# bioinformatics-centre/kaiju

Hardware: AMD Instinct MI355X
Metric: classified reads/sec (150 bp) (higher is better)
Workload: dtype u64

## Files before the change

### kaiju_amd/csrc/capi.hip

```cpp
#include <algorithm>
#include <chrono>
#include <cstdio>
#include <cstring>
#include <memory>
#include <thread>

#include "capi_internal.h"
#include "host_tables.h"
#include "kj_flow.h"
#include "taxonomy.h"
#include "exact_pass.h"
#include "kj_format.h"
#ifdef KJ_GREEDY3
#include "kj_greedy3.h"
#endif

using namespace kj;

constexpr uint32_t kLocDeferRows = 8;

__device__ __forceinline__ void load_tables(ConstTables &s_ct, const ConstTables *g_ct) {
  const uint32_t *src = reinterpret_cast<const uint32_t *>(g_ct);
  uint32_t *dst = reinterpret_cast<uint32_t *>(&s_ct);
  for (uint32_t i = threadIdx.x; i < sizeof(ConstTables) / 4; i += kBlock) dst[i] = src[i];
// ... 113 lines not shown
      }
      F[k].flags = fl;
    }
    b.meta[r].nfrag = nf | pending;
    uint64_t *h8 = reinterpret_cast<uint64_t *>(b.hits + r);
    for (int x = 0; x < (int)(sizeof(Hit) / 8); x++) h8[x] = 0;
  }
}
__global__ void __launch_bounds__(kBlock)
k_seg_apply_list(const ConstTables *__restrict__ g_ct, Params p, Batch b, SegQueue sq, const uint32_t *seglist,
                 const uint32_t *segcount, uint32_t *err) {
  __shared__ ConstTables s_ct;
  load_tables(s_ct, g_ct);
  const uint32_t n = *segcount;
  uint32_t e = 0;
  for (uint32_t i = blockIdx.x * kBlock + threadIdx.x; i < n; i += gridDim.x * kBlock) seg_apply_mem(s_ct, p, b, sq, seglist[i], &e);
  if (e) atomicOr(err, e);
}

#ifdef KJ_POST_WAVES
#define KJ_POST_BOUNDS __launch_bounds__(256, KJ_POST_WAVES)
#else
#define KJ_POST_BOUNDS __launch_bounds__(256)
#endif
template <bool LCA>
__global__ void KJ_POST_BOUNDS
k_mem_post1(const Stage1Tables *__restrict__ g_t, DevIndex ix, Params p, Batch b, DevTaxonomy t, CompactHit *__restrict__ compact, int lazy,
            uint32_t *seglist, uint32_t *segcount, uint32_t *todo, uint32_t *todocount) {
  __shared__ __attribute__((aligned(16))) Stage1Tables s_t;
  __shared__ __attribute__((aligned(4))) uint8_t s_cnt[256 * kS1CntStride];
  if (lazy) {
    const uint4 *src = reinterpret_cast<const uint4 *>(g_t);
    uint4 *dst = reinterpret_cast<uint4 *>(&s_t);
    for (uint32_t i = threadIdx.x; i < sizeof(Stage1Tables) / 16; i += 256) dst[i] = src[i];
    __syncthreads();
  }
  const uint32_t r = blockIdx.x * 256 + threadIdx.x;
  bool need = false, later = false;
  if (r < b.n_reads) {
    Hit *h = b.hits + r;
    const uint32_t v = lazy ? h->reserved : 0u;
    if (v != 0) {
      h->reserved = 0;
#ifndef KJ_POST_NOTRIG
      need = lazy_seg_needed(s_t, p, b, r, h, v, nullptr, s_cnt + threadIdx.x * kS1CntStride);
#endif
    }
    if (!need) {
      if (h->flags & kHitRetry) later = true;
#ifdef KJ_POST_NOLOCATE
      else if (LCA) { CompactHit ch; ch.lca = 0; ch.best = h->best; ch.info = 0; compact[r] = ch; }
#else
      else if (!mem_locate_read<false>(ix, p, h, kLocDeferRows)) later = true;
      else if (LCA) compact[r] = compact_hit(t, *h);
#endif
    }
  }
  const uint32_t lane = threadIdx.x & 63u;
  {
    const uint64_t m = __ballot(need);
    if (m) {
      const uint32_t leader = (uint32_t)__builtin_ctzll(m);
      uint32_t base = 0;
      if (lane == leader) base = atomicAdd(segcount, (uint32_t)__popcll(m));
      base = (uint32_t)__shfl((int)base, (int)leader, 64);
      if (need) seglist[base + (uint32_t)__popcll(m & ((1ull << lane) - 1ull))] = r;
    }
  }
  {
    const bool td = need || later;
    const uint64_t m = __ballot(td);
    if (m) {
      const uint32_t leader = (uint32_t)__builtin_ctzll(m);
      uint32_t base = 0;
      if (lane == leader) base = atomicAdd(todocount, (uint32_t)__popcll(m));
      base = (uint32_t)__shfl((int)base, (int)leader, 64);
      if (td) todo[base + (uint32_t)__popcll(m & ((1ull << lane) - 1ull))] = r;
    }
  }
}
template <bool LCA>
__global__ void __launch_bounds__(256)
k_mem_post2(DevIndex ix, Params p, Batch b, DevTaxonomy t, CompactHit *__restrict__ compact, const uint32_t *__restrict__ todo,
            const uint32_t *__restrict__ todocount) {
  const uint32_t n = *todocount;
  for (uint32_t i = blockIdx.x * 256 + threadIdx.x; i < n; i += gridDim.x * 256) {
    const uint32_t r = todo[i];
    Hit *h = b.hits + r;
    if (!mem_locate_read<false>(ix, p, h, kLocDeferRows)) mem_locate_read<false, true>(ix, p, h);
    if (LCA) compact[r] = compact_hit(t, *h);
  }
}

__global__ void __launch_bounds__(kFragBlock)
k_fragments_protein(const ConstTables *__restrict__ g_ct, Params p, SegTables st, Batch b, SegQueue sq, uint32_t *err) {
  __shared__ ConstTables s_ct;
  __shared__ int32_t s_entg[17];
  __shared__ uint8_t s_code[256];
  if (threadIdx.x < 17) s_entg[threadIdx.x] = st.ent_g32[threadIdx.x];
  {
    const uint32_t *src = reinterpret_cast<const uint32_t *>(g_ct);
    uint32_t *dst = reinterpret_cast<uint32_t *>(&s_ct);
    for (uint32_t i = threadIdx.x; i < sizeof(ConstTables) / 4; i += kFragBlock) dst[i] = src[i];
    for (uint32_t i = threadIdx.x; i < 256; i += kFragBlock) s_code[i] = 0;
    __syncthreads();
    if (threadIdx.x < 20) protein_code_entry(s_ct, threadIdx.x, s_code);
    __syncthreads();
// ... 418 lines not shown
    for (int x = threadIdx.x & 63; x < 2 + 3 * PS_N; x += 64) s_prof[threadIdx.x >> 6][x] = 0;
    gx.prof = s_prof[threadIdx.x >> 6];
    if ((threadIdx.x & 63) == 0) { gx.prof[0] = __builtin_readcyclecounter(); gx.prof[1] = PS_HEAD; }
  }
#endif
  greedy_lane3<COUNT>(ix, s_ct, p, sq, b, wl, gx);
}
__global__ void __launch_bounds__(kG3Threads, 2)
k_greedy3(DevIndex ix, const ConstTables *__restrict__ g_ct, Params p, SegQueue sq, Batch b, WorkList wl, GreedyArrays2 ga, uint32_t split) {
  greedy3_body<false>(ix, g_ct, p, sq, b, wl, ga, split);
}
__global__ void __launch_bounds__(kG3Threads, 2)
k_greedy3_count(DevIndex ix, const ConstTables *__restrict__ g_ct, Params p, SegQueue sq, Batch b, WorkList wl, GreedyArrays2 ga, uint32_t split) {
  greedy3_body<true>(ix, g_ct, p, sq, b, wl, ga, split);
}

#endif

static_assert(sizeof(ConstTables) % 4 == 0, "ConstTables is copied as dwords");
static_assert(sizeof(Hit) == sizeof(kaiju_gpu_hit), "hit layout");

static thread_local std::string tl_error;
int fail(int code, const std::string &msg) { tl_error = msg; return code; }

extern "C" int kaiju_gpu_abi_version(void) { return KAIJU_GPU_ABI_VERSION; }
extern "C" const char *kaiju_gpu_last_error(void) { return tl_error.c_str(); }
extern "C" void kj_set_last_error(const char *msg) { tl_error = msg ? msg : ""; }
extern "C" const char *kaiju_gpu_strerror(int status) {
  switch (status) {
    case KAIJU_GPU_OK: return "ok";
    case KAIJU_GPU_ERR_ARG: return "bad argument";
    case KAIJU_GPU_ERR_IO: return "I/O error";
    case KAIJU_GPU_ERR_FORMAT: return "unrecognised file content";
    case KAIJU_GPU_ERR_NO_DEVICE: return "no usable HIP device (this library has no CPU path)";
    case KAIJU_GPU_ERR_HIP: return "HIP runtime error";
    case KAIJU_GPU_ERR_NOMEM: return "out of memory";
    case KAIJU_GPU_ERR_UNSUPPORTED: return "parameter not supported by the kernels";
    case KAIJU_GPU_ERR_INDEX_BUG: return "index triggers a latent bug of the reference";
    default: return "unknown status";
  }
}
extern "C" int kaiju_gpu_device_count(void) {
  int n = 0;
  if (hipGetDeviceCount(&n) != hipSuccess) return 0;
  return n;
}
int no_device() {
  int ndev = 0;
  if (hipGetDeviceCount(&ndev) != hipSuccess || ndev <= 0) return fail(KAIJU_GPU_ERR_NO_DEVICE, "hipGetDeviceCount found no device");
  return KAIJU_GPU_OK;
}

__global__ void __launch_bounds__(256)
k_lca(DevTaxonomy t, const Hit *__restrict__ hits, uint32_t n, CompactHit *__restrict__ out) {
  const uint32_t r = blockIdx.x * 256 + threadIdx.x;
  if (r >= n) return;
  out[r] = compact_hit(t, hits[r]);
}
int launch_lca(hipStream_t s, const kaiju_gpu_taxonomy *t, const kaiju_gpu_hit *d_hits, uint32_t n, kaiju_gpu_compact *d_out) {
  hipLaunchKernelGGL(k_lca, dim3((n + 255) / 256), dim3(256), 0, s, t->dev, reinterpret_cast<const Hit *>(d_hits), n,
                     reinterpret_cast<CompactHit *>(d_out));
  KJ_HIP(hipGetLastError());
  return KAIJU_GPU_OK;
}

int ensure(DevBuf &b, size_t bytes) {
  if (bytes <= b.cap) return 0;
  if (b.p) { KJ_HIP(hipFree(b.p)); b.p = nullptr; b.cap = 0; }
  const size_t want = bytes + bytes / 8 + 256;
  KJ_HIP(hipMalloc(&b.p, want));
  b.cap = want;
  return 0;
}

extern "C" void kaiju_gpu_default_params(kaiju_gpu_params *p, int mode) {
  if (!p) return;
  p->mode = mode ? 1 : 0;
  p->min_fragment_length = 11;
  p->mismatches = 3;
  p->min_score = 65;
  p->seed_length = 7;
  p->seg = 1;
  p->use_evalue = mode ? 1 : 0;
  p->min_evalue = 0.01;
  p->max_matches_SI = 20;
  p->max_match_ids = 20;
  p->input_is_protein = 0;
}

extern "C" int kaiju_gpu_create(kaiju_gpu_ctx **out, const kaiju_gpu_index *ix, const kaiju_gpu_params *p) {
  return guarded([&]() -> int {
  if (!out || !ix || !p) return fail(KAIJU_GPU_ERR_ARG, "NULL argument");
  *out = nullptr;
  if (p->mode != 0 && p->mode != 1) return fail(KAIJU_GPU_ERR_ARG, "mode must be 0 (MEM) or 1 (GREEDY)");
  if (p->min_fragment_length < 1 || p->min_fragment_length > 10000)
    return fail(KAIJU_GPU_ERR_UNSUPPORTED, "min_fragment_length out of range");
  if (p->mode == 1 && p->mismatches > (uint32_t)kMaxMismatch)
    return fail(KAIJU_GPU_ERR_UNSUPPORTED, "more than 8 mismatches are not supported");
  if (p->mode == 1 && p->seed_length < 1) return fail(KAIJU_GPU_ERR_ARG, "seed_length must be >= 1");
  if (p->max_match_ids > 20 || p->max_matches_SI > 64 || p->max_matches_SI < 1)
    return fail(KAIJU_GPU_ERR_UNSUPPORTED, "max_match_ids <= 20 and 1 <= max_matches_SI <= 64 required");
  std::unique_ptr<kaiju_gpu_ctx> c(new kaiju_gpu_ctx());
  c->ix = ix;
  c->params = *p;
  c->kp.mode = p->mode; c->kp.m = p->min_fragment_length; c->kp.mismatches = p->mismatches;
  c->kp.min_score = p->min_score; c->kp.seed_length = p->seed_length; c->kp.seg = p->seg ? 1 : 0;
  c->kp.max_matches_SI = p->max_matches_SI; c->kp.max_match_ids = p->max_match_ids;
  if (const char *e = getenv("KAIJU_GPU_DEBUG")) c->kp.debug = (uint32_t)atoi(e);
  if (const char *e = getenv("KAIJU_GPU_EXACT_PASS")) c->exact_pass = atoi(e) != 0;
  if (const char *e = getenv("KAIJU_GPU_MEM_LANE")) c->mem_v1 = !strcmp(e, "v1");
  if (const char *e = getenv("KAIJU_GPU_VERBOSE_LANE")) c->verbose_v1 = !strcmp(e, "v1");
  c->dump_frags = getenv("KAIJU_GPU_DUMP_FRAGS");
  if (const char *e = getenv("KAIJU_GPU_STAGE1")) { c->stage1_old = !strcmp(e, "old"); c->stage1_lane = !strcmp(e, "lane"); }
  if (const char *e = getenv("KAIJU_GPU_LAZY_SEG")) c->lazy_seg = atoi(e) != 0;
// ... 379 lines not shown
      g2.bestv = nullptr; g2.vb = vb;
      if (c->verbose) {
        if ((rc = ensure(c->vb_bestv, lanes_g2 * 64 * sizeof(GBestV)))) return rc;
        g2.bestv = static_cast<GBestV *>(c->vb_bestv.p);
      }
    }
    call_mark("launch_batch: Greedy scratch in place");
    if (plan.run) {
      const dim3 grid(c->blocks_main);
      const bool counting = plan.inst == FlowInst::Counting;
      switch (plan.lane) {
        case FlowLane::Greedy2Wide:
          if (plan.inst == FlowInst::Verbose) hipLaunchKernelGGL(k_greedy2_wide_vb, grid, blk, kGreedy2Lds, s, ix->dev, ix->d_ct, p_lane, sq, b, wl_main, g2);
          else if (counting) hipLaunchKernelGGL(k_greedy2_wide_count, grid, blk, kGreedy2Lds, s, ix->dev, ix->d_ct, p_lane, sq, b, wl_main, g2);
          else hipLaunchKernelGGL(k_greedy2_wide, grid, blk, kGreedy2Lds, s, ix->dev, ix->d_ct, p_lane, sq, b, wl_main, g2);
          break;
#ifdef KJ_GREEDY3
        case FlowLane::Greedy3:
          if (counting) hipLaunchKernelGGL(k_greedy3_count, dim3(c->n_cu), dim3(c->g3_threads), 0, s, ix->dev, ix->d_ct, p_lane, sq, b, wl_main, g2, c->g3_split);
          else hipLaunchKernelGGL(k_greedy3, dim3(c->n_cu), dim3(c->g3_threads), 0, s, ix->dev, ix->d_ct, p_lane, sq, b, wl_main, g2, c->g3_split);
          break;
#else
        case FlowLane::Greedy3:
#endif
        case FlowLane::Greedy2:
          if (plan.inst == FlowInst::Verbose) hipLaunchKernelGGL(k_greedy2_vb, grid, blk, kGreedy2Lds, s, ix->dev, ix->d_ct, p_lane, sq, b, wl_main, g2);
          else if (counting) hipLaunchKernelGGL(k_greedy2_count, grid, blk, kGreedy2Lds, s, ix->dev, ix->d_ct, p_lane, sq, b, wl_main, g2);
          else hipLaunchKernelGGL(k_greedy2, grid, blk, kGreedy2Lds, s, ix->dev, ix->d_ct, p_lane, sq, b, wl_main, g2);
          break;
        case FlowLane::GreedyV1:
          hipLaunchKernelGGL(k_greedy, grid, blk, 0, s, ix->dev, ix->d_ct, p, sq, b, wl_main, ga, vb);
          break;
        default: break;
      }
      KJ_HIP(hipGetLastError());
      KJ_HIP(hipEventRecord(c->ev[3], s));
      hipLaunchKernelGGL(k_greedy_retry, dim3(c->blocks_retry), blk, 0, s, ix->dev, ix->d_ct, p, sq, b, wl_retry, gr, vb);
      KJ_HIP(hipGetLastError());
      if (plan.mem_verbose) {
        hipLaunchKernelGGL(pick_greedy_verbose(lane_wide), grid_reads, dim3(256), 0, s, ix->dev, p, b, vb);
        KJ_HIP(hipGetLastError());
      }
      launch_locate(c, s, plan.locate, p, b, loc_list, cnt + kCntLocListGreedy);
      KJ_HIP(hipGetLastError());
      if (plan.exact_pass) {
        xp.g_pool = gr.pool; xp.g_ord = gr.ord; xp.g_matches = gr.matches; xp.g_best = gr.best; xp.g_bestv = gr.bestv;
        xp.g_pool_cap = gr.pool_cap; xp.g_match_cap = gr.match_cap; xp.blocks_search = c->blocks_retry;
        xp.vb = vb;
        KJ_HIP(kj_launch_exact_pass(xp));
      }
    } else KJ_HIP(hipEventRecord(c->ev[3], s));
  }
  if (plan.lca) {
    hipLaunchKernelGGL(k_lca, dim3((n + 255) / 256), dim3(256), 0, s, tax->dev, reinterpret_cast<const Hit *>(d_out), n,
                       reinterpret_cast<CompactHit *>(d_compact));
    KJ_HIP(hipGetLastError());
  }
  KJ_HIP(hipEventRecord(c->ev[4], s));
  c->ev_valid = true;
  c->last_n = n;
  if (const char *dump = c->dump_frags) {
    KJ_HIP(hipStreamSynchronize(s));
    std::vector<ReadMeta> hm(n);
    KJ_HIP(hipMemcpy(hm.data(), c->meta.p, (size_t)n * sizeof(ReadMeta), hipMemcpyDeviceToHost));
    std::vector<uint8_t> hp(c->pep.cap);
    KJ_HIP(hipMemcpy(hp.data(), c->pep.p, c->pep.cap, hipMemcpyDeviceToHost));
    std::vector<uint8_t> hf(c->frags.cap);
    KJ_HIP(hipMemcpy(hf.data(), c->frags.p, c->frags.cap, hipMemcpyDeviceToHost));
    const Frag *F = reinterpret_cast<const Frag *>(hf.data());
    if (FILE *fp = fopen(dump, "a")) {
      const char *alpha = ix->info.alphabet;
      for (uint32_t r = 0; r < n; r++) {
        fprintf(fp, "#\n");
        for (uint32_t k = 0; k < (hm[r].nfrag & ~kNfragSegPending); k++) {
          const Frag &f = F[hm[r].frag + k];
          fprintf(fp, "%u:", f.key);
          for (uint32_t x = 0; x < f.len; x++) fputc(alpha[hp[hm[r].pep + f.start + x] % 21], fp);
          fprintf(fp, "\n");
        }
      }
      fclose(fp);
    }
  }
  return KAIJU_GPU_OK;
}

extern "C" int kaiju_gpu_classify_batch_device(kaiju_gpu_ctx *ctx, const void *d_seqs, uint64_t seq_bytes,
                                               const uint64_t *d_off, uint32_t n_reads, int paired,
                                               kaiju_gpu_hit *d_out, void *stream) {
  return guarded([&]() -> int {
  if (!ctx || (!d_seqs && seq_bytes) || !d_off || (!d_out && n_reads)) return fail(KAIJU_GPU_ERR_ARG, "NULL argument");
  KJ_HIP(hipSetDevice(ctx->ix->device));
  hipStream_t s = stream ? static_cast<hipStream_t>(stream) : ctx->stream;
  return launch_batch(ctx, d_seqs, seq_bytes, d_off, n_reads, paired, ctx->max_read_len, d_out, s);
  });
}

int classify_host_buffers(kaiju_gpu_ctx *ctx, const char *seqs, const uint64_t *off, uint32_t n_reads, int paired,
                          const kaiju_gpu_taxonomy *tax) {
  KJ_HIP(hipSetDevice(ctx->ix->device));
  if (off[0] != 0) return fail(KAIJU_GPU_ERR_ARG, "off[0] must be 0");
  const uint64_t seq_bytes = off[2 * (uint64_t)n_reads];
  uint32_t max_len = 0;
  for (uint64_t i = 0; i < 2 * (uint64_t)n_reads; i++) {
    if (off[i + 1] < off[i]) return fail(KAIJU_GPU_ERR_ARG, "offsets must be non-decreasing");
    const uint64_t l = off[i + 1] - off[i];
    if (l > 0x3fffffffull) return fail(KAIJU_GPU_ERR_UNSUPPORTED, "read longer than 2^30");
    if (l > max_len) max_len = (uint32_t)l;
  }
// ... 37 lines not shown
  });
}

extern "C" int kaiju_gpu_set_max_read_length(kaiju_gpu_ctx *ctx, uint32_t max_read_len) {
  if (!ctx || max_read_len == 0 || max_read_len > 0x3fffffffu) return fail(KAIJU_GPU_ERR_ARG, "bad max_read_len");
  ctx->max_read_len = max_read_len;
  return KAIJU_GPU_OK;
}

extern "C" int kaiju_gpu_taxonomy_upload(const kaiju_taxonomy *t, int device_id, kaiju_gpu_taxonomy **out) {
  return guarded([&]() -> int {
  if (!t || !out) return fail(KAIJU_GPU_ERR_ARG, "NULL argument");
  *out = nullptr;
  int ndev = 0;
  if (hipGetDeviceCount(&ndev) != hipSuccess || ndev <= 0)
    return fail(KAIJU_GPU_ERR_NO_DEVICE, "hipGetDeviceCount found no device");
  if (device_id < 0 || device_id >= ndev) return fail(KAIJU_GPU_ERR_ARG, "device_id out of range");
  std::vector<uint64_t> key, parent_id;
  std::vector<uint32_t> parent_slot, depth;
  kj_taxonomy_table(t, key, parent_id, parent_slot, depth);
  std::unique_ptr<kaiju_gpu_taxonomy> g(new kaiju_gpu_taxonomy());
  g->device = device_id;
  KJ_HIP(hipSetDevice(device_id));
  auto up = [&](const void *src, size_t bytes, const void **dst) -> int {
    void *p = nullptr;
    KJ_HIP(hipMalloc(&p, bytes + 16));
    g->allocs.push_back(p);
    KJ_HIP(hipMemcpy(p, src, bytes, hipMemcpyHostToDevice));
    *dst = p;
    return 0;
  };
  int rc;
  if ((rc = up(key.data(), key.size() * 8, (const void **)&g->dev.key))) return rc;
  if ((rc = up(parent_id.data(), parent_id.size() * 8, (const void **)&g->dev.parent_id))) return rc;
  if ((rc = up(parent_slot.data(), parent_slot.size() * 4, (const void **)&g->dev.parent_slot))) return rc;
  if ((rc = up(depth.data(), depth.size() * 4, (const void **)&g->dev.depth))) return rc;
  g->dev.cap_mask = (uint32_t)(key.size() - 1);
  *out = g.release();
  return KAIJU_GPU_OK;
  });
}

extern "C" void kaiju_gpu_taxonomy_free(kaiju_gpu_taxonomy *t) { delete t; }

static_assert(sizeof(CompactHit) == sizeof(kaiju_gpu_compact) && sizeof(CompactHit) == 16, "compact record layout");

extern "C" int kaiju_gpu_lca_batch_device(kaiju_gpu_ctx *ctx, const kaiju_gpu_taxonomy *t, const kaiju_gpu_hit *d_hits,
                                          uint32_t n_reads, kaiju_gpu_compact *d_out, void *stream) {
  if (!ctx || !t || (!d_hits && n_reads) || (!d_out && n_reads)) return fail(KAIJU_GPU_ERR_ARG, "NULL argument");
  if (t->device != ctx->ix->device) return fail(KAIJU_GPU_ERR_ARG, "taxonomy lives on another device");
  if (n_reads == 0) return KAIJU_GPU_OK;
  KJ_HIP(hipSetDevice(ctx->ix->device));
  hipStream_t s = stream ? static_cast<hipStream_t>(stream) : ctx->stream;
  return launch_lca(s, t, d_hits, n_reads, d_out);
}

int verbose_queue(kaiju_gpu_ctx *ctx, const char *seqs, const uint64_t *off, uint32_t n_reads, int paired) {
  ctx->verbose = true;
  int rc = classify_host_buffers(ctx, seqs, off, n_reads, paired);
  ctx->verbose = false;
  if (rc) return rc;
  call_mark("verbose: launch_batch returned");
  hipStream_t s = ctx->stream;
  const char *alpha = ctx->ix->info.alphabet;
  VbAlphabet al{};
  al.n = (uint32_t)std::min<size_t>(strlen(alpha), sizeof al.c);
  memcpy(al.c, alpha, al.n);
  if ((rc = ensure(ctx->vb_packed, (size_t)n_reads * ctx->vb_text_cap + 16))) return rc;
  if ((rc = ensure(ctx->vb_pos, (size_t)n_reads * 8 + 16))) return rc;
  VerboseOut vbd{static_cast<uint32_t *>(ctx->vb_nacc.p), static_cast<uint32_t *>(ctx->vb_acc.p), static_cast<uint32_t *>(ctx->vb_tlen.p),
                 static_cast<uint8_t *>(ctx->vb_text.p), ctx->vb_text_cap};
  unsigned long long *d_total = reinterpret_cast<unsigned long long *>(static_cast<uint8_t *>(ctx->vb_pos.p) + (size_t)n_reads * 8);
  KJ_HIP(hipMemsetAsync(d_total, 0, 8, s));
  hipLaunchKernelGGL(k_vb_pack, dim3((n_reads + 255) / 256), dim3(256), 0, s, vbd, n_reads, al, static_cast<uint8_t *>(ctx->vb_packed.p),
                     static_cast<uint64_t *>(ctx->vb_pos.p), d_total);
  KJ_HIP(hipGetLastError());
  return KAIJU_GPU_OK;
}
static int verbose_core(kaiju_gpu_ctx *ctx, const char *seqs, const uint64_t *off, uint32_t n_reads, int paired, kaiju_gpu_hit *out,
                        kaiju_gpu_verbose *vout, std::vector<uint64_t> &pos, std::vector<uint32_t> &tlen) {
  int rc = verbose_queue(ctx, seqs, off, n_reads, paired);
  if (rc) return rc;
  hipStream_t s = ctx->stream;
  std::vector<uint32_t> &nacc = ctx->vb_h_nacc, &acc = ctx->vb_h_acc;
  if (nacc.size() < n_reads) nacc.resize(n_reads);
  if (acc.size() < (size_t)n_reads * kVbAcc) acc.resize((size_t)n_reads * kVbAcc);
  pos.resize((size_t)n_reads + 1); tlen.resize(n_reads);
  KJ_HIP(hipMemcpyAsync(out, ctx->h_hits.p, (size_t)n_reads * sizeof(kaiju_gpu_hit), hipMemcpyDeviceToHost, s));
  KJ_HIP(hipMemcpyAsync(nacc.data(), ctx->vb_nacc.p, (size_t)n_reads * 4, hipMemcpyDeviceToHost, s));
  KJ_HIP(hipMemcpyAsync(tlen.data(), ctx->vb_tlen.p, (size_t)n_reads * 4, hipMemcpyDeviceToHost, s));
  KJ_HIP(hipMemcpyAsync(acc.data(), ctx->vb_acc.p, (size_t)n_reads * kVbAcc * 4, hipMemcpyDeviceToHost, s));
  KJ_HIP(hipMemcpyAsync(pos.data(), ctx->vb_pos.p, ((size_t)n_reads + 1) * 8, hipMemcpyDeviceToHost, s));
  call_mark("verbose: everything queued");
  KJ_HIP(hipStreamSynchronize(s));
  call_mark("verbose: stream drained (records, accessions, positions on the host)");
  const uint64_t total = pos[n_reads];
  if (total > (uint64_t)n_reads * ctx->vb_text_cap) return fail(KAIJU_GPU_ERR_HIP, "k_vb_pack: impossible total");
  if (ctx->vb_host.size() < total) ctx->vb_host.resize((size_t)total);
  if (total) KJ_HIP(hipMemcpy(ctx->vb_host.data(), ctx->vb_packed.p, (size_t)total, hipMemcpyDeviceToHost));
  for (uint32_t r = 0; r < n_reads; r++) {
    kaiju_gpu_verbose &v = vout[r];
    v.n_acc = nacc[r] > (uint32_t)kVbAcc ? (uint32_t)kVbAcc : nacc[r];
    for (uint32_t q = 0; q < (uint32_t)KAIJU_GPU_MAX_ACC; q++) v.acc_iseq[q] = q < v.n_acc ? acc[(size_t)r * kVbAcc + q] : 0;
    v.text_len = tlen[r] < ctx->vb_text_cap ? tlen[r] : ctx->vb_text_cap;
    v.truncated = tlen[r] > ctx->vb_text_cap ? 1u : 0u;
  }
  return KAIJU_GPU_OK;
// ... 463 lines not shown
```

### kaiju_amd/csrc/capi_internal.h

```cpp
#pragma once
#include <hip/hip_runtime.h>

#include <new>
#include <stdexcept>
#include <string>
#include <vector>

#include "../../include/kaiju_gpu.h"
#include "kj_core.h"
#include "kj_lines.h"

namespace kjv { struct Job; }
namespace kjq { struct Job; }

#pragma GCC visibility push(hidden)
int fail(int code, const std::string &msg);
#define KJ_HIP(call)                                                                         \
  do {                                                                                       \
    hipError_t e_ = (call);                                                                  \
    if (e_ != hipSuccess)                                                                    \
      return fail(KAIJU_GPU_ERR_HIP, std::string(#call) + ": " + hipGetErrorString(e_));     \
  } while (0)

template <class F>
// ... 30 lines not shown
  const uint8_t *sn_blob = nullptr;
  const uint64_t *sn_off = nullptr;
  const uint32_t *sn_len = nullptr;
  uint64_t sn_bytes = 0;
  uint32_t sn_max = 0;
  bool sn_ready = false;
  ~kaiju_gpu_index() {
    (void)hipSetDevice(device);
    for (void *p : allocs) (void)hipFree(p);
  }
};

struct kaiju_gpu_taxonomy {
  int device = 0;
  kj::DevTaxonomy dev{};
  std::vector<void *> allocs;
  ~kaiju_gpu_taxonomy() {
    (void)hipSetDevice(device);
    for (void *p : allocs) (void)hipFree(p);
  }
};

struct DevBuf {
  void *p = nullptr;
  size_t cap = 0;
};

struct kaiju_gpu_ctx {
  const kaiju_gpu_index *ix = nullptr;
  kaiju_gpu_params params{};
  kj::Params kp{};
  hipStream_t stream = nullptr;
  hipEvent_t ev[6] = {nullptr, nullptr, nullptr, nullptr, nullptr, nullptr};
  bool ev_valid = false;
  int n_cu = 0, blocks_main = 0, blocks_retry = 0;
  DevBuf pep, frags, meta, counters, retry_list, seg_items, seg_recs;
  DevBuf scratch_main[10], scratch_retry[5], h_compact;
  DevBuf redo_bitmap, redo_list, redo_items, redo_index, redo_pool, redo_work, redo_cls;
  bool greedy2 = false;
  bool greedy3 = false;
  uint32_t g3_split = 1;
  uint32_t g3_threads = 512;
  uint32_t g1_pool = 192, g1_match = 64;
  bool g1_pool_set = false;
  uint32_t greedy_gate = 1u | 32u << 8;
  bool verbose = false;
  bool exact_pass = true;
  bool count_ops = false;
  bool mem_v1 = false;
  bool verbose_v1 = false;
  bool stage1_old = false;
  bool stage1_lane = false;
  bool lazy_seg = true;
  DevBuf seglist, loc_list, todo_list;
  int seg_team = 64;
  bool fused_post = true;
  const char *dump_frags = nullptr;
  uint32_t vb_text_cap = 0;
  DevBuf vb_nacc, vb_acc, vb_tlen, vb_text, vb_bestv, vb_bestv_retry;
  DevBuf vb_packed, vb_pos;
  std::vector<uint8_t> vb_host;
  std::vector<uint32_t> vb_h_nacc, vb_h_acc;
  DevBuf h_seqs, h_off, h_hits;
  kjl::Scratch ingest;
  DevBuf ing_text1, ing_text2, ing_names, ing_info;
  kjl::Lines format;
  DevBuf fmt_pw, fmt_out, fmt_info;
  bool fmt_pw_ok = false;
  kjl::Lines format_v;
  DevBuf fv_out, fv_info, fv_trunc;
  kjl::Lines format_s;
  kjl::Lines format_n;
  kaiju_gpu_stats stats{};
  uint32_t last_n = 0;
  uint32_t max_read_len = 1024;
  ~kaiju_gpu_ctx() {
    if (!ix) return;
    (void)hipSetDevice(ix->device);
    ingest.release();
    for (kjl::Lines *l : {&format, &format_v, &format_s, &format_n}) l->release();
    DevBuf *all[] = {&fv_out, &fv_info, &fv_trunc, &fmt_pw, &fmt_out, &fmt_info, &ing_text1, &ing_text2, &ing_names, &ing_info, &pep, &frags, &meta, &counters, &retry_list, &seg_items, &seg_recs, &h_seqs, &h_off, &h_hits, &h_compact, &seglist, &loc_list, &todo_list,
                     &vb_nacc, &vb_acc, &vb_tlen, &vb_text, &vb_bestv, &vb_bestv_retry, &vb_packed, &vb_pos,
                     &redo_bitmap, &redo_list, &redo_items, &redo_index, &redo_pool, &redo_work, &redo_cls};
    for (DevBuf *b : all) if (b->p) (void)hipFree(b->p);
    for (int i = 0; i < 10; i++) if (scratch_main[i].p) (void)hipFree(scratch_main[i].p);
    for (int i = 0; i < 5; i++) if (scratch_retry[i].p) (void)hipFree(scratch_retry[i].p);
    for (auto &e : ev) if (e) (void)hipEventDestroy(e);
    if (stream) (void)hipStreamDestroy(stream);
  }
};

int ensure(DevBuf &b, size_t bytes);

int classify_host_buffers(kaiju_gpu_ctx *ctx, const char *seqs, const uint64_t *off, uint32_t n_reads, int paired,
                          const kaiju_gpu_taxonomy *tax = nullptr);
int verbose_queue(kaiju_gpu_ctx *ctx, const char *seqs, const uint64_t *off, uint32_t n_reads, int paired);
int launch_lca(hipStream_t s, const kaiju_gpu_taxonomy *t, const kaiju_gpu_hit *d_hits, uint32_t n, kaiju_gpu_compact *d_out);

bool index_accessions(const kaiju_gpu_index *ix, kjv::Job &J);
bool index_seq_names(const kaiju_gpu_index *ix, kjq::Job &J);
int no_format_verbose();
int no_format_seq();
#pragma GCC visibility pop
```

### kaiju_amd/csrc/capi_text.hip

```cpp
#include <algorithm>
#include <cstring>
#include <type_traits>

#include "capi_internal.h"
#include "kj_ingest.h"
#include "kj_format.h"
#include "kj_format_verbose.h"
#include "kj_format_seq.h"
#include "kj_format_names.h"
__attribute__((weak)) decltype(kj_ingest_launch) kj_ingest_launch;
__attribute__((weak)) decltype(kj_format_launch) kj_format_launch;
__attribute__((weak)) decltype(kj_fv_lengths) kj_fv_lengths;
__attribute__((weak)) decltype(kj_fv_write) kj_fv_write;
extern "C" __attribute__((weak)) decltype(kaiju_accession_ranks) kaiju_accession_ranks;
__attribute__((weak)) decltype(kj_fs_lengths) kj_fs_lengths;
__attribute__((weak)) decltype(kj_fs_write) kj_fs_write;
__attribute__((weak)) decltype(kj_fn_launch) kj_fn_launch;
__attribute__((weak)) decltype(kj_fn_device) kj_fn_device;
extern "C" __attribute__((weak)) decltype(kaiju_gpu_taxon_names_max_annotation) kaiju_gpu_taxon_names_max_annotation;

using namespace kj;

static int no_ingest() { return kj_ingest_launch ? KAIJU_GPU_OK : fail(KAIJU_GPU_ERR_UNSUPPORTED, "this library was linked without ingest.hip"); }

// ... 392 lines not shown
  if (int rc = no_format_verbose()) return rc;
  if (!ctx || !info || (n && (!hits || !vout || !text_pos || !recs || !off || !names)) || (!text && text_bytes) || (!names_text && names_bytes) ||
      (!out && out_cap)) return fail(KAIJU_GPU_ERR_ARG, "NULL argument");
  if (names_bytes > kjf::kMaxBytes || n > kjf::kMaxRecords) return fail(KAIJU_GPU_ERR_ARG, "the names must be below 2^32 - 32 bytes, a batch below 2^31 records");
  KJ_HIP(hipSetDevice(ctx->ix->device));
  kjv::Job J{};
  int rc;
  if ((rc = fv_job(ctx, paired, J))) return rc;
  if ((rc = stage_peptides(ctx, vout, text_pos, text, text_bytes, text_cap, n, true))) return rc;
  if ((rc = ensure(ctx->h_hits, ((size_t)n + 1) * sizeof(kaiju_gpu_hit)))) return rc;
  if ((rc = ensure(ctx->h_compact, ((size_t)n + 1) * sizeof(kaiju_gpu_compact)))) return rc;
  if ((rc = ensure(ctx->h_off, (2 * (size_t)n + 1) * 8))) return rc;
  if ((rc = stage_names(ctx, names_text, names_bytes, names, n))) return rc;
  if ((rc = ensure(ctx->fv_out, out_cap + 64))) return rc;
  if ((rc = ensure(ctx->fv_info, sizeof(kaiju_gpu_format_verbose_info)))) return rc;
  hipStream_t s = ctx->stream;
  if (n) {
    KJ_HIP(hipMemcpyAsync(ctx->h_hits.p, hits, (size_t)n * sizeof(kaiju_gpu_hit), hipMemcpyHostToDevice, s));
    KJ_HIP(hipMemcpyAsync(ctx->h_compact.p, recs, (size_t)n * sizeof(kaiju_gpu_compact), hipMemcpyHostToDevice, s));
    KJ_HIP(hipMemcpyAsync(ctx->h_off.p, off, (2 * (size_t)n + 1) * 8, hipMemcpyHostToDevice, s));
  }
  bind_records(ctx, J, names_bytes);
  bind_peptides(ctx, J, text_cap, true);
  const char *err = "";
  rc = kj_fv_lengths(ctx->format_v, s, J, n, &err);
  if (rc == 0) rc = kj_fv_write(ctx->format_v, s, J, n, ctx->fv_out.p, out_cap, static_cast<kaiju_gpu_format_verbose_info *>(ctx->fv_info.p), &err);
  if (rc) { (void)hipStreamSynchronize(s); return fail(rc, err); }
  return format_download(s, ctx->format_v, ctx->fv_info, ctx->fv_out, out, out_cap, info);
  });
}

extern "C" int kaiju_gpu_classify_batch_verbose_text(kaiju_gpu_ctx *ctx, const kaiju_gpu_taxonomy *t, const char *seqs, const uint64_t *off,
                                                     uint32_t n_reads, int paired, const char *names_text, uint64_t names_bytes,
                                                     const kaiju_gpu_name_span *names, const char **text, uint64_t *text_bytes,
                                                     kaiju_gpu_format_verbose_info *info) {
  return guarded([&]() -> int {
  if (int rc = no_device()) return rc;
  if (int rc = no_format_verbose()) return rc;
  if (!ctx || !t || !off || !text || !text_bytes || !info || (n_reads && !names) || (!names_text && names_bytes)) return fail(KAIJU_GPU_ERR_ARG, "NULL argument");
  if (t->device != ctx->ix->device) return fail(KAIJU_GPU_ERR_ARG, "taxonomy lives on another device");
  if (names_bytes > kjf::kMaxBytes || n_reads > kjf::kMaxRecords) return fail(KAIJU_GPU_ERR_ARG, "the names must be below 2^32 - 32 bytes, a batch below 2^31 records");
  *text = nullptr; *text_bytes = 0;
  memset(info, 0, sizeof *info);
  if (n_reads == 0) return KAIJU_GPU_OK;
  KJ_HIP(hipSetDevice(ctx->ix->device));
  kjv::Job J{};
  int rc;
  if ((rc = fv_job(ctx, paired, J))) return rc;
  if ((rc = stage_names(ctx, names_text, names_bytes, names, n_reads))) return rc;
  if ((rc = ensure(ctx->h_compact, ((size_t)n_reads + 1) * sizeof(kaiju_gpu_compact)))) return rc;
  if ((rc = ensure(ctx->fv_info, sizeof(kaiju_gpu_format_verbose_info)))) return rc;
  hipStream_t s = ctx->stream;
  if ((rc = verbose_queue(ctx, seqs, off, n_reads, paired))) return rc;
  if ((rc = launch_lca(s, t, static_cast<const kaiju_gpu_hit *>(ctx->h_hits.p), n_reads, static_cast<kaiju_gpu_compact *>(ctx->h_compact.p)))) return rc;
  bind_records(ctx, J, names_bytes);
  bind_peptides(ctx, J, ctx->vb_text_cap, false);
  const char *err = "";
  if ((rc = kj_fv_lengths(ctx->format_v, s, J, n_reads, &err))) return fail(rc, err);
  return write_sized_text(ctx, ctx->format_v, names_bytes + (uint64_t)n_reads * (512 + 20ull * (kjv::kMaxPrefix + 1) + ctx->vb_text_cap),
                          "verbose text: size of the text on the host", [&](uint64_t total, const char **e) {
    return kj_fv_write(ctx->format_v, s, J, n_reads, ctx->fv_out.p, total, static_cast<kaiju_gpu_format_verbose_info *>(ctx->fv_info.p), e);
  }, text, text_bytes, info);
  });
}

int no_format_seq() { return kj_fs_lengths ? KAIJU_GPU_OK : fail(KAIJU_GPU_ERR_UNSUPPORTED, "this library was linked without format_seq.hip"); }

static int fs_job(kaiju_gpu_ctx *ctx, int paired, int u_rule, kjq::Job &J) {
  if (ctx->ix->id_mode != KAIJU_GPU_IDS_SEQUENCE) return fail(KAIJU_GPU_ERR_ARG, "the lines of kaijux / kaijup need an index loaded with KAIJU_GPU_IDS_SEQUENCE");
  if (u_rule != KAIJU_GPU_U_RULE_NUCLEOTIDE && u_rule != KAIJU_GPU_U_RULE_PROTEIN) return fail(KAIJU_GPU_ERR_ARG, "u_rule must be KAIJU_GPU_U_RULE_NUCLEOTIDE or KAIJU_GPU_U_RULE_PROTEIN");
  if (int rc = format_params(ctx, paired, J.P)) return rc;
  if (!index_seq_names(ctx->ix, J)) return fail(KAIJU_GPU_ERR_ARG, "the index has no sequence-name table on the device: call kaiju_gpu_index_upload_seq_names() first");
  J.nseq = (uint32_t)ctx->ix->names.size();
  J.pw = static_cast<const double *>(ctx->fmt_pw.p);
  J.u_rule = (uint32_t)u_rule;
  J.min_frag = ctx->params.min_fragment_length;
  J.min_score = ctx->params.min_score;
  J.greedy = ctx->params.mode == 0 ? 0u : 1u;
  return KAIJU_GPU_OK;
}

extern "C" int kaiju_gpu_format_seq_device(kaiju_gpu_ctx *ctx, const kaiju_gpu_hit *d_hits, const uint64_t *d_off, uint32_t n, int paired,
                                           int u_rule, const void *d_seqs, const uint64_t *d_text_pos, const uint32_t *d_text_len,
                                           const void *d_pep, uint32_t text_cap, const void *d_names_text, uint64_t names_bytes,
                                           const kaiju_gpu_name_span *d_names, void *d_out, uint64_t out_cap,
                                           kaiju_gpu_format_verbose_info *d_info, void *stream) {
  return guarded([&]() -> int {
  if (int rc = no_device()) return rc;
  if (int rc = no_format_seq()) return rc;
  if (!ctx || !d_info || (!d_out && out_cap)) return fail(KAIJU_GPU_ERR_ARG, "NULL argument");
  if ((uintptr_t)d_out & 15) return fail(KAIJU_GPU_ERR_ARG, "the output pointer must be 16-byte aligned");
  KJ_HIP(hipSetDevice(ctx->ix->device));
  kjq::Job J{};
  if (int rc = fs_job(ctx, paired, u_rule, J)) return rc;
  J.hits = d_hits; J.off = d_off; J.seqs = static_cast<const uint8_t *>(d_seqs);
  J.pep = static_cast<const uint8_t *>(d_pep);
  if (d_pep) { J.text_pos = d_text_pos; J.text_len = d_text_len; J.text_cap = text_cap; }
  J.names_text = static_cast<const uint8_t *>(d_names_text); J.names_bytes = names_bytes; J.names = d_names;
  hipStream_t s = stream ? static_cast<hipStream_t>(stream) : ctx->stream;
  const char *err = "";
  int rc = kj_fs_lengths(ctx->format_s, s, J, n, &err);
  if (rc) return fail(rc, err);
  rc = kj_fs_write(ctx->format_s, s, J, n, d_out, out_cap, d_info, &err);
  return rc ? fail(rc, err) : KAIJU_GPU_OK;
  });
}

// ... 79 lines not shown
```

### kaiju_amd/csrc/kj_core.h

```cpp
#pragma once
#include <type_traits>
#include <stdint.h>

#if defined(__HIPCC__)
#include <hip/hip_runtime.h>
#define KJ_HD __host__ __device__ __forceinline__
#define KJ_HD_NOINLINE __host__ __device__ __noinline__
#else
#define KJ_HD inline
#define KJ_HD_NOINLINE inline
struct uint2 { uint32_t x, y; };
struct ulonglong2 { uint64_t x, y; };
#endif

namespace kj {

struct u128 { uint64_t x, y; };
typedef u128 u128_unaligned __attribute__((aligned(1)));
typedef uint32_t u32_unaligned __attribute__((aligned(1)));
typedef uint64_t u64_unaligned __attribute__((aligned(1)));

constexpr int kMaxIds = 21;
constexpr int kSbShift = 16;
constexpr uint32_t kHitIdCap = 1u, kHitSiCap = 2u;
constexpr uint32_t kHitInternalOverflow = 0x80000000u;
constexpr uint32_t kHitRetry = 0x40000000u;
constexpr uint32_t kHitLocPending = 0x20000000u;
constexpr int kWin = 64, kWinStride = 68;
constexpr int kLocWideShift = 40;
constexpr uint32_t kLocWideMaxLen = 1u << 24;

struct alignas(128) RankBlock64 {
  uint64_t plane[5];
  uint32_t cnt[20];
  uint32_t pad[2];
};
static_assert(sizeof(RankBlock64) == 128, "RankBlock64 must be one 128-byte line");

struct DevIndex {
  const RankBlock64 *blocks64;
  const uint64_t *mb_base;
  uint32_t mb_shift;
  const uint64_t *sa_taxid;
  const uint32_t *sa_iseq;
  const uint64_t *seq_taxid;
  const uint8_t *seq_valid;
  const uint64_t *term_pos;
  uint64_t C[22];
  uint64_t bwtlen;
  uint64_t n_sa;
  uint64_t sa_skip;
  uint32_t nseq;
  uint32_t chpt_exp;
  const uint2 *kmer32;
  const ulonglong2 *kmer64;
  uint32_t kmer_k;
  const uint8_t *kline;
  uint32_t kline_k;
  const uint32_t *sa_full;
  const uint8_t *text;
  const uint32_t *row_tax;
  const uint64_t *tax_of_dense;
  uint32_t n_dense;
  uint32_t beyond_lo, beyond_n, beyond_row;
  const uint8_t *sa_tpos5;
  uint32_t tv_shift;
  const uint32_t *row_tax_s = nullptr;
  uint32_t rts_shift = 0;
};
constexpr uint64_t kTposNone = (1ull << 40) - 1ull;
constexpr uint32_t kBeyondRowsMax = 4096;
constexpr uint32_t kTextPad = 64;
#ifndef KJ_TEXT_CMP
#define KJ_TEXT_CMP 48
#endif
// ... 4533 lines not shown
struct DevTaxonomy {
  const uint64_t *key;
  const uint64_t *parent_id;
  const uint32_t *parent_slot;
  const uint32_t *depth;
  uint32_t cap_mask;
};
struct CompactHit {
  uint64_t lca;
  uint32_t best;
  uint32_t info;
};
KJ_HD uint32_t tax_hash(uint64_t id) {
  id ^= id >> 33; id *= 0xff51afd7ed558ccdULL; id ^= id >> 33; id *= 0xc4ceb9fe1a85ec53ULL; id ^= id >> 33;
  return (uint32_t)id;
}
KJ_HD uint32_t tax_find(const DevTaxonomy &t, uint64_t id) {
  uint32_t s = tax_hash(id) & t.cap_mask;
  for (;;) {
    const uint64_t k = t.key[s];
    if (k == id) return s;
    if (k == ~0ull) return ~0u;
    s = (s + 1) & t.cap_mask;
  }
}
KJ_HD uint64_t tax_lca(const DevTaxonomy &t, const uint64_t *ids, uint32_t n) {
  if (n == 0) return 0;
  if (n == 1) return ids[0];
  uint64_t leaf[kMaxIds];
  uint32_t slot[kMaxIds], dep[kMaxIds];
  uint32_t m = 0, shallowest = 0xffffffffu;
  for (uint32_t i = 0; i < n && i < (uint32_t)kMaxIds; i++) {
    const uint32_t s = tax_find(t, ids[i]);
    if (s == ~0u) continue;
    leaf[m] = ids[i]; slot[m] = s; dep[m] = t.depth[s];
    if (dep[m] < shallowest) shallowest = dep[m];
    m++;
  }
  if (m == 0) return 0;
  for (uint32_t i = 0; i < m; i++)
    for (uint32_t d = dep[i]; d > shallowest; d--)
      if (slot[i] != ~0u) { leaf[i] = t.parent_id[slot[i]]; slot[i] = t.parent_slot[slot[i]]; }
  for (uint32_t step = 0; step <= shallowest + 1; step++) {
    const uint64_t first = leaf[0];
    bool same = true;
    for (uint32_t i = 0; i < m; i++) {
      if (leaf[i] != first) same = false;
      if (slot[i] != ~0u) { leaf[i] = t.parent_id[slot[i]]; slot[i] = t.parent_slot[slot[i]]; }
    }
    if (same) return first;
  }
  return 0;
}
KJ_HD CompactHit compact_hit(const DevTaxonomy &t, const Hit &h) {
  CompactHit c;
  c.best = h.best; c.info = h.flags << 8 | (h.flags & kHitInternalOverflow) | (h.n_ids & 255u);
  c.lca = (h.n_ids == 0 || h.best == 0) ? 0 : tax_lca(t, h.taxid, h.n_ids);
  return c;
}

}
```

Baseline: 474.9 million.

## Split LCA into register-resident small-set fast path and compacted general fallback

Adds a templated LCA routine for reads with at most three taxon ids that keeps leaves, slots and depths in unrolled registers instead of generic arrays. The standalone LCA kernel handles small sets inline and pushes the remaining reads onto a list via wave ballot and atomics, which a second grid-stride kernel then processes with the general path. The aim is to cut divergence and register/scratch pressure in the common case. In exchange it adds an extra kernel launch, a memset and a list buffer, and the fused post kernel is switched to the general routine.

```diff
diff --git a/kaiju_amd/csrc/capi.hip b/kaiju_amd/csrc/capi.hip
--- a/kaiju_amd/csrc/capi.hip
+++ b/kaiju_amd/csrc/capi.hip
@@ -189,7 +189,7 @@
       else if (LCA) { CompactHit ch; ch.lca = 0; ch.best = h->best; ch.info = 0; compact[r] = ch; }
 #else
       else if (!mem_locate_read<false>(ix, p, h, kLocDeferRows)) later = true;
-      else if (LCA) compact[r] = compact_hit(t, *h);
+      else if (LCA) compact[r] = compact_hit_general(t, *h);
 #endif
     }
   }
@@ -714,14 +714,46 @@
 }
 
 __global__ void __launch_bounds__(256)
-k_lca(DevTaxonomy t, const Hit *__restrict__ hits, uint32_t n, CompactHit *__restrict__ out) {
+k_lca(DevTaxonomy t, const Hit *__restrict__ hits, uint32_t n, CompactHit *__restrict__ out, uint32_t *list, uint32_t *listcount) {
   const uint32_t r = blockIdx.x * 256 + threadIdx.x;
-  if (r >= n) return;
-  out[r] = compact_hit(t, hits[r]);
-}
-int launch_lca(hipStream_t s, const kaiju_gpu_taxonomy *t, const kaiju_gpu_hit *d_hits, uint32_t n, kaiju_gpu_compact *d_out) {
-  hipLaunchKernelGGL(k_lca, dim3((n + 255) / 256), dim3(256), 0, s, t->dev, reinterpret_cast<const Hit *>(d_hits), n,
-                     reinterpret_cast<CompactHit *>(d_out));
+  bool later = false;
+  if (r < n) {
+    const Hit *h = hits + r;
+    LocIds li;
+    li.n_ids = h->n_ids; li.flags = h->flags;
+#pragma unroll
+    for (int q = 0; q < kLcaSmallIds; q++) li.id[q] = (uint32_t)q < li.n_ids ? h->taxid[q] : 0ull;
+    CompactHit ch;
+    if (compact_hit_small(t, h->best, li, &ch)) out[r] = ch;
+    else later = true;
+  }
+  const uint64_t m = __ballot(later);
+  if (m) {
+    const uint32_t lane = threadIdx.x & 63u, leader = (uint32_t)__builtin_ctzll(m);
+    uint32_t base = 0;
+    if (lane == leader) base = atomicAdd(listcount, (uint32_t)__popcll(m));
+    base = (uint32_t)__shfl((int)base, (int)leader, 64);
+    if (later) list[base + (uint32_t)__popcll(m & ((1ull << lane) - 1ull))] = r;
+  }
+}
+__global__ void __launch_bounds__(256)
+k_lca_list(DevTaxonomy t, const Hit *__restrict__ hits, CompactHit *__restrict__ out, const uint32_t *__restrict__ list,
+           const uint32_t *__restrict__ listcount) {
+  const uint32_t n = *listcount;
+  for (uint32_t i = blockIdx.x * 256 + threadIdx.x; i < n; i += gridDim.x * 256) out[list[i]] = compact_hit(t, hits[list[i]]);
+}
+int launch_lca(kaiju_gpu_ctx *ctx, hipStream_t s, const kaiju_gpu_taxonomy *t, const kaiju_gpu_hit *d_hits, uint32_t n, kaiju_gpu_compact *d_out) {
+  if (n == 0) return KAIJU_GPU_OK;
+  int rc;
+  if ((rc = ensure(ctx->lca_list, ((size_t)n + 4) * 4))) return rc;
+  uint32_t *const count = static_cast<uint32_t *>(ctx->lca_list.p), *const list = count + 4;
+  KJ_HIP(hipMemsetAsync(count, 0, 4, s));
+  const uint32_t blocks = (n + 255) / 256;
+  hipLaunchKernelGGL(k_lca, dim3(blocks), dim3(256), 0, s, t->dev, reinterpret_cast<const Hit *>(d_hits), n,
+                     reinterpret_cast<CompactHit *>(d_out), list, count);
+  KJ_HIP(hipGetLastError());
+  hipLaunchKernelGGL(k_lca_list, dim3(std::min<uint32_t>(blocks, (uint32_t)ctx->n_cu * 4u)), dim3(256), 0, s, t->dev,
+                     reinterpret_cast<const Hit *>(d_hits), reinterpret_cast<CompactHit *>(d_out), list, count);
   KJ_HIP(hipGetLastError());
   return KAIJU_GPU_OK;
 }
@@ -1207,9 +1239,7 @@
     } else KJ_HIP(hipEventRecord(c->ev[3], s));
   }
   if (plan.lca) {
-    hipLaunchKernelGGL(k_lca, dim3((n + 255) / 256), dim3(256), 0, s, tax->dev, reinterpret_cast<const Hit *>(d_out), n,
-                       reinterpret_cast<CompactHit *>(d_compact));
-    KJ_HIP(hipGetLastError());
+    if ((rc = launch_lca(c, s, tax, d_out, n, d_compact))) return rc;
   }
   KJ_HIP(hipEventRecord(c->ev[4], s));
   c->ev_valid = true;
@@ -1353,7 +1383,7 @@
   if (n_reads == 0) return KAIJU_GPU_OK;
   KJ_HIP(hipSetDevice(ctx->ix->device));
   hipStream_t s = stream ? static_cast<hipStream_t>(stream) : ctx->stream;
-  return launch_lca(s, t, d_hits, n_reads, d_out);
+  return launch_lca(ctx, s, t, d_hits, n_reads, d_out);
 }
 
 int verbose_queue(kaiju_gpu_ctx *ctx, const char *seqs, const uint64_t *off, uint32_t n_reads, int paired) {
diff --git a/kaiju_amd/csrc/capi_internal.h b/kaiju_amd/csrc/capi_internal.h
--- a/kaiju_amd/csrc/capi_internal.h
+++ b/kaiju_amd/csrc/capi_internal.h
@@ -106,7 +106,7 @@
   bool stage1_old = false;
   bool stage1_lane = false;
   bool lazy_seg = true;
-  DevBuf seglist, loc_list, todo_list;
+  DevBuf seglist, loc_list, todo_list, lca_list;
   int seg_team = 64;
   bool fused_post = true;
   const char *dump_frags = nullptr;
@@ -133,7 +133,7 @@
     (void)hipSetDevice(ix->device);
     ingest.release();
     for (kjl::Lines *l : {&format, &format_v, &format_s, &format_n}) l->release();
-    DevBuf *all[] = {&fv_out, &fv_info, &fv_trunc, &fmt_pw, &fmt_out, &fmt_info, &ing_text1, &ing_text2, &ing_names, &ing_info, &pep, &frags, &meta, &counters, &retry_list, &seg_items, &seg_recs, &h_seqs, &h_off, &h_hits, &h_compact, &seglist, &loc_list, &todo_list,
+    DevBuf *all[] = {&fv_out, &fv_info, &fv_trunc, &fmt_pw, &fmt_out, &fmt_info, &ing_text1, &ing_text2, &ing_names, &ing_info, &pep, &frags, &meta, &counters, &retry_list, &seg_items, &seg_recs, &h_seqs, &h_off, &h_hits, &h_compact, &seglist, &loc_list, &todo_list, &lca_list,
                      &vb_nacc, &vb_acc, &vb_tlen, &vb_text, &vb_bestv, &vb_bestv_retry, &vb_packed, &vb_pos,
                      &redo_bitmap, &redo_list, &redo_items, &redo_index, &redo_pool, &redo_work, &redo_cls};
     for (DevBuf *b : all) if (b->p) (void)hipFree(b->p);
@@ -149,7 +149,7 @@
 int classify_host_buffers(kaiju_gpu_ctx *ctx, const char *seqs, const uint64_t *off, uint32_t n_reads, int paired,
                           const kaiju_gpu_taxonomy *tax = nullptr);
 int verbose_queue(kaiju_gpu_ctx *ctx, const char *seqs, const uint64_t *off, uint32_t n_reads, int paired);
-int launch_lca(hipStream_t s, const kaiju_gpu_taxonomy *t, const kaiju_gpu_hit *d_hits, uint32_t n, kaiju_gpu_compact *d_out);
+int launch_lca(kaiju_gpu_ctx *ctx, hipStream_t s, const kaiju_gpu_taxonomy *t, const kaiju_gpu_hit *d_hits, uint32_t n, kaiju_gpu_compact *d_out);
 
 bool index_accessions(const kaiju_gpu_index *ix, kjv::Job &J);
 bool index_seq_names(const kaiju_gpu_index *ix, kjq::Job &J);
diff --git a/kaiju_amd/csrc/capi_text.hip b/kaiju_amd/csrc/capi_text.hip
--- a/kaiju_amd/csrc/capi_text.hip
+++ b/kaiju_amd/csrc/capi_text.hip
@@ -468,7 +468,7 @@
   if ((rc = ensure(ctx->fv_info, sizeof(kaiju_gpu_format_verbose_info)))) return rc;
   hipStream_t s = ctx->stream;
   if ((rc = verbose_queue(ctx, seqs, off, n_reads, paired))) return rc;
-  if ((rc = launch_lca(s, t, static_cast<const kaiju_gpu_hit *>(ctx->h_hits.p), n_reads, static_cast<kaiju_gpu_compact *>(ctx->h_compact.p)))) return rc;
+  if ((rc = launch_lca(ctx, s, t, static_cast<const kaiju_gpu_hit *>(ctx->h_hits.p), n_reads, static_cast<kaiju_gpu_compact *>(ctx->h_compact.p)))) return rc;
   bind_records(ctx, J, names_bytes);
   bind_peptides(ctx, J, ctx->vb_text_cap, false);
   const char *err = "";
diff --git a/kaiju_amd/csrc/kj_core.h b/kaiju_amd/csrc/kj_core.h
--- a/kaiju_amd/csrc/kj_core.h
+++ b/kaiju_amd/csrc/kj_core.h
@@ -21,6 +21,7 @@
 typedef uint64_t u64_unaligned __attribute__((aligned(1)));
 
 constexpr int kMaxIds = 21;
+constexpr int kLcaSmallIds = 3;
 constexpr int kSbShift = 16;
 constexpr uint32_t kHitIdCap = 1u, kHitSiCap = 2u;
 constexpr uint32_t kHitInternalOverflow = 0x80000000u;
@@ -4660,11 +4661,75 @@
   }
   return 0;
 }
-KJ_HD CompactHit compact_hit(const DevTaxonomy &t, const Hit &h) {
+template <int K>
+KJ_HD bool tax_lca_small(const DevTaxonomy &t, const uint64_t (&ids)[K], uint32_t n, uint64_t *lca) {
+  static_assert(K >= 2 && K <= kMaxIds, "a small set");
+  if (n > (uint32_t)K) return false;
+  if (n == 0) { *lca = 0; return true; }
+  if (n == 1) { *lca = ids[0]; return true; }
+  uint64_t leaf[K];
+  uint32_t slot[K], dep[K];
+  uint64_t leaf_f = 0;
+  uint32_t slot_f = ~0u, dep_f = 0;
+#pragma unroll
+  for (int i = 0; i < K; i++) {
+    leaf[i] = 0; dep[i] = 0;
+    slot[i] = (uint32_t)i < n ? tax_find(t, ids[i]) : ~0u;
+    if (slot[i] != ~0u) {
+      leaf[i] = ids[i]; dep[i] = t.depth[slot[i]];
+      if (slot_f == ~0u) { leaf_f = leaf[i]; slot_f = slot[i]; dep_f = dep[i]; }
+    }
+  }
+  if (slot_f == ~0u) { *lca = 0; return true; }
+  uint32_t shallowest = dep_f;
+#pragma unroll
+  for (int i = 0; i < K; i++) {
+    if (slot[i] == ~0u) { leaf[i] = leaf_f; slot[i] = slot_f; dep[i] = dep_f; }
+    if (dep[i] < shallowest) shallowest = dep[i];
+  }
+#pragma unroll
+  for (int i = 0; i < K; i++)
+    for (uint32_t d = dep[i]; d > shallowest; d--)
+      if (slot[i] != ~0u) { leaf[i] = t.parent_id[slot[i]]; slot[i] = t.parent_slot[slot[i]]; }
+  for (uint32_t step = 0; step <= shallowest + 1; step++) {
+    const uint64_t first = leaf[0];
+    bool same = true;
+#pragma unroll
+    for (int i = 0; i < K; i++) {
+      if (leaf[i] != first) same = false;
+      if (slot[i] != ~0u) { leaf[i] = t.parent_id[slot[i]]; slot[i] = t.parent_slot[slot[i]]; }
+    }
+    if (same) { *lca = first; return true; }
+  }
+  *lca = 0;
+  return true;
+}
+struct LocIds {
+  uint32_t n_ids, flags;
+  uint64_t id[kLcaSmallIds];
+};
+KJ_HD bool compact_hit_small(const DevTaxonomy &t, uint32_t best, const LocIds &l, CompactHit *c) {
+  uint64_t lca = 0;
+  if (l.n_ids != 0 && best != 0 && !tax_lca_small<kLcaSmallIds>(t, l.id, l.n_ids, &lca)) return false;
+  c->lca = lca; c->best = best; c->info = l.flags << 8 | (l.flags & kHitInternalOverflow) | (l.n_ids & 255u);
+  return true;
+}
+KJ_HD CompactHit compact_hit_general(const DevTaxonomy &t, const Hit &h) {
   CompactHit c;
   c.best = h.best; c.info = h.flags << 8 | (h.flags & kHitInternalOverflow) | (h.n_ids & 255u);
   c.lca = (h.n_ids == 0 || h.best == 0) ? 0 : tax_lca(t, h.taxid, h.n_ids);
   return c;
 }
-
-}
+KJ_HD CompactHit compact_hit(const DevTaxonomy &t, const Hit &h) {
+  CompactHit c;
+  LocIds l;
+  l.n_ids = h.n_ids; l.flags = h.flags;
+#pragma unroll
+  for (int i = 0; i < kLcaSmallIds; i++) l.id[i] = (uint32_t)i < h.n_ids ? h.taxid[i] : 0ull;
+  if (compact_hit_small(t, h.best, l, &c)) return c;
+  c.best = h.best; c.info = h.flags << 8 | (h.flags & kHitInternalOverflow) | (h.n_ids & 255u);
+  c.lca = tax_lca(t, h.taxid, h.n_ids);
+  return c;
+}
+
+}
```

Result: no change. 475.8 million (median of 4 runs) (+0.2%).
